# dohlee/diffab-pytorch

Hardware: AMD Instinct MI355X
Metric: CDR-residue denoise-steps/sec (K=128 patch) (higher is better)
Workload: dtype f32 (bf16x6 / fp16x3 split-precision products on the 16-bit matrix cores, fp32 accumulate; fp32-accurate, DESIGN section 4)

## Files before the change

### diffab-pytorch_amd/csrc/api.hip

```cpp
#include <atomic>
#include <cstring>
#include <mutex>
#include <vector>

#include "common.h"
#include "denoiser_internal.h"
#include "mlp_chain_tile.h"

namespace diffab {

static thread_local char g_err[512] = "";

void set_error(const char* fmt, ...) {
  va_list ap;
  va_start(ap, fmt);
  vsnprintf(g_err, sizeof(g_err), fmt, ap);
  va_end(ap);
}

namespace {
struct OrderState {
  std::recursive_mutex mu;
  hipStream_t last = nullptr;
  bool have = false;
// ... 132 lines not shown
  if (hipGetDevice(&dev) == hipSuccess) (void)hipDeviceGetAttribute(&ncu, hipDeviceAttributeMultiprocessorCount, dev);
  const int rounds = (d->B + ncu - 1) / ncu;
  return d->K == 128 && d->B >= ncu && static_cast<double>(d->B) >= 0.85 * rounds * ncu;
}

struct ForwardPlan {
  uint32_t flags;
  bool fold;
  bool b6;
  bool chain;
  bool persistent, fused_mlps;
  const float* pair_planes;
  const int* ctx_of_row;
  int n_ctx;
  const unsigned char* last_layer_tiles;
  float* res_emb;
};

static ForwardPlan plan_forward(const diffab_dims* d, uint32_t flags, const StepBuffers& b, const float* res_ctx, const float* pair_ctx,
                                float* res_emb, bool loop, const int* ctx_of_row = nullptr, int n_ctx = 0, unsigned char* tiles = nullptr) {
  const int rows = d->B * d->K, D = d->D;
  if (loop && !(flags & DIFFAB_FLAG_PAIR_F32)) flags |= DIFFAB_FLAG_PAIR_PLANES;
  ForwardPlan p{};
  p.flags = flags;
  p.fold = !(flags & DIFFAB_FLAG_FORCE_GENERIC) && fast_path_supported(d) && rowgemm128_ok(res_ctx, D, b.h1, D, rows, D);
  p.b6 = p.fold && use_b6_gemm(flags) && rowgemm128_b6_ok(res_ctx, D, b.h1, D, rows, D);
  p.chain = p.b6 && d->V <= 128;
  p.pair_planes = use_pair_planes(d, flags, pair_ctx, b) ? b.pair : nullptr;
  p.ctx_of_row = ctx_of_row;
  p.n_ctx = n_ctx;
  p.last_layer_tiles = tiles != nullptr && !(flags & DIFFAB_FLAG_ALL_ROWS) && p.fold && d->K % 16 == 0 && d->NL >= 2 ? tiles : nullptr;
  p.res_emb = res_emb;
  p.persistent = p.b6 && p.pair_planes != nullptr && ipa_module_persistent_supported(d) &&
                 ((flags & DIFFAB_FLAG_PERSISTENT_MODULE) || (loop && !(flags & DIFFAB_FLAG_MULTI_LAUNCH) && module_launch_fills_chip(d)));
  p.fused_mlps = p.persistent && p.chain && D == 128 && res_emb == nullptr;
  return p;
}

struct StepBias {
  const float* beta;
  const float* sched_beta;
  int t;
  const int* t_dev;
  float* beta_traj;
  int traj_rows;
};

static int prepare_forward(const diffab_dims* d, const diffab_denoiser_weights* w, const ForwardPlan& p, const StepBuffers& b,
                           const float* pair_ctx, const StepBias& bias, hipStream_t st) {
  if (p.fold)
// ... 62 lines not shown
  const int head_div = bias.beta_traj ? rows : d->K;
  if (p.chain) {
    for (int hd = 0; hd < 3; ++hd) {
      hpl[3 * hd] = mlp + (2 + 2 * hd) * mlp_planes_bytes();
      hpl[3 * hd + 1] = mlp + (3 + 2 * hd) * mlp_planes_bytes();
      hpl[3 * hd + 2] = mlp + (8 + hd) * mlp_planes_bytes();
      hbs[3 * hd] = bias.beta_traj ? bias.beta_traj + (static_cast<size_t>(hd) * bias.traj_rows + bias.t) * D
                                   : b.beta_tab + static_cast<size_t>(hd) * d->B * D;
      hbs[3 * hd + 1] = hw[hd]->b2;
      hbs[3 * hd + 2] = hw[hd]->b4;
    }
    if (int rc = make_mlp_chain_set(&head_set, 3, hpl, hbs, nullptr, head_div, 3, nout, outs, nout)) return rc;
  }
  if (p.persistent) {
    if (int rc = launch_ipa_module_persistent(d, b.hA, b.hB, O_t, x_t, b.ipa, b.planes, p.pair_planes, st, p.fused_mlps ? res_ctx : nullptr,
                                              &emb_set, &head_set, p.ctx_of_row, p.n_ctx, p.last_layer_tiles))
      return rc;
    cur = (d->NL & 1) ? b.hB : b.hA;
  }
  for (int l = 0; l < d->NL && !p.persistent; ++l) {
    const void* planes = p.b6 ? b.planes + l * ipa_layer_planes_bytes() : nullptr;
    if (int rc = ipa_layer_dispatch(d, &w->layers[l], cur, pair_ctx, O_t, x_t, nxt, b.ipa, p.flags, st, nullptr, nullptr, planes, p.pair_planes,
                                    false, l == d->NL - 1 ? p.last_layer_tiles : nullptr, p.ctx_of_row, p.n_ctx))
      return rc;
    float* tmp = cur; cur = nxt; nxt = tmp;
  }
  if (p.res_emb) DIFFAB_HIP_CHECK(hipMemcpyAsync(p.res_emb, cur, sizeof(float) * rows * D, hipMemcpyDeviceToDevice, st));
  if (p.chain) {
    if (!p.fused_mlps)
      if (int rc = launch_mlp_chains_b6(cur, D, 3, hpl, hbs, nullptr, head_div, 3, nout, outs, nout, rows, st)) return rc;
  } else if (p.fold) {
// ... 37 lines not shown
  float* outs[3] = {out_eps, tp.vbuf, tp.logits};
  const int nout[3] = {3, 3, d->V};
  for (int hd = 0; hd < 3; ++hd) {
    if (int rc = launch_linear(tp.cat3, D + 3, hw[hd]->w0, hw[hd]->b0, tp.t1[hd], D, rows, D, D + 3, true, st)) return rc;
    if (int rc = launch_linear(tp.t1[hd], D, hw[hd]->w2, hw[hd]->b2, tp.t2[hd], D, rows, D, D, true, st)) return rc;
    if (int rc = launch_linear(tp.t2[hd], D, hw[hd]->w4, hw[hd]->b4, outs[hd], nout[hd], rows, nout[hd], D, false, st)) return rc;
  }
  return launch_heads_finish(tp.vbuf, O_t, tp.logits, d->V, rows, out_O0, out_post, st);
}

constexpr int kTrajRows = 1025;
struct SampleBuffers {
  float *beta, *eps, *O0, *post;
  int* t_dev;
  unsigned char* tiles;
  float* beta_traj;
  int* ctx_of_row;
  float* res_ctx;
  void* step;
  size_t bytes;
};

static SampleBuffers carve_sample(const diffab_dims* d, void* ws, int n_pair = 0, bool mapped = false) {
  Carver c(ws);
  const size_t rows = static_cast<size_t>(d->B) * d->K;
  SampleBuffers s;
  s.beta = c.take<float>(d->B);
  s.eps = c.take<float>(rows * 3);
  s.O0 = c.take<float>(rows * 9);
  s.post = c.take<float>(rows * d->V);
  s.t_dev = c.take<int>(64);
  s.tiles = c.take<unsigned char>(static_cast<size_t>(d->B) * ((d->K + 15) / 16));
  s.beta_traj = c.take<float>(static_cast<size_t>(3) * kTrajRows * d->D);
  s.ctx_of_row = mapped ? c.take<int>(d->B) : nullptr;
  s.res_ctx = mapped ? c.take<float>(rows * d->D) : nullptr;
  const size_t step_bytes = carve_step(d, nullptr, n_pair).bytes;
  s.step = c.take<char>(step_bytes);
  s.bytes = c.bytes();
  return s;
}

struct ScoreBuffers {
  int* t_list;
  float* beta;
  int* ctx_of_row;
  int64_t* seq_t;
  float *x_t, *O_t, *eps, *eps_hat;
// ... 87 lines not shown

int diffab_debug_set_module_stagger(int32_t ticks_10ns, int32_t classes) {
  set_module_stagger(ticks_10ns, classes);
  return DIFFAB_OK;
}

int diffab_debug_set_module_stamps(void* device_buffer) {
  set_module_stamps(device_buffer);
  return DIFFAB_OK;
}

int diffab_debug_row_tiles(const uint8_t* gen_mask, int32_t B, int32_t K, uint8_t* tiles, void* stream) {
  StreamOrder order_(stream);
  DIFFAB_REQUIRE(gen_mask && tiles && B >= 1 && K >= 16 && K % 16 == 0, DIFFAB_ERR_ARG, "debug_row_tiles: need B >= 1 and K a multiple of 16");
  return launch_tiles_needed(gen_mask, B, K, tiles, as_stream(stream));
}

int diffab_debug_set_attn_variant(int32_t v) { return set_attn_variant(v); }

int diffab_debug_set_attn_stamps(void* device_buffer) {
  set_attn_stamps(device_buffer);
  return DIFFAB_OK;
}

int diffab_kernel_timer_enable(int on) {
  g_timer.on = on != 0;
  g_timer.used = 0;
  return DIFFAB_OK;
}

// ... 429 lines not shown
  const bool mapped = ctx_of_row != nullptr;
  int n_ctx = opt->n_ctx;
  bool identity = false;
  if (int rc = context_map_option(d, ctx_of_row, &n_ctx, &identity)) return rc;
  const SampleBuffers sb = carve_sample(d, workspace, n_ctx, mapped);
  DIFFAB_REQUIRE(workspace_bytes >= sb.bytes, DIFFAB_ERR_WORKSPACE, "sample_loop: workspace %zu < %zu bytes", workspace_bytes, sb.bytes);
  hipStream_t st = as_stream(stream);
  const int* ctx_dev = nullptr;
  if (!identity) {
    DIFFAB_HIP_CHECK(hipMemcpyAsync(sb.ctx_of_row, ctx_of_row, sizeof(int32_t) * d->B, hipMemcpyHostToDevice, st));
    if (int rc = launch_gather_rows(res_ctx, sb.ctx_of_row, d->B, static_cast<int64_t>(d->K) * d->D, sb.res_ctx, st)) return rc;
    ctx_dev = sb.ctx_of_row;
    res_ctx = sb.res_ctx;
  }
  const StepBuffers b0 = carve_step(d, sb.step, n_ctx);
  const ForwardPlan plan = plan_forward(d, flags, b0, res_ctx, pair_ctx, nullptr, true, ctx_dev, n_ctx, sb.tiles);
  StepBias bias{sb.beta, plan.fold ? s->beta : nullptr, 0, nullptr, nullptr, s->T + 1};
  if (plan.chain && s->T + 1 <= kTrajRows && !(flags & DIFFAB_FLAG_GRAPH_SAMPLER)) bias.beta_traj = sb.beta_traj;
  if (int rc = prepare_forward(d, w, plan, b0, pair_ctx, bias, st)) return rc;
  if (plan.last_layer_tiles)
    if (int rc = launch_tiles_needed(gen_mask, d->B, d->K, sb.tiles, st)) return rc;
  if (rec != nullptr) {
    DIFFAB_HIP_CHECK(hipMemcpyAsync(rec->slot_dev, rec->slot_of_step, sizeof(int32_t) * (s->T + 1), hipMemcpyHostToDevice, st));
    if (int rc = launch_record_fixed(uo.rec, seq, x, O, gen_mask, d->B, d->K, d->V, st)) return rc;
  }
  if (steps != nullptr)
    DIFFAB_HIP_CHECK(hipMemcpyAsync(steps->plan_dev, plan_host.data(), sizeof(int32_t) * plan_host.size(), hipMemcpyHostToDevice, st));
  if (steering != nullptr && steering->ancestors != nullptr)
    DIFFAB_HIP_CHECK(hipMemsetAsync(steering->ancestors, 0xFF, sizeof(int32_t) * static_cast<size_t>(s->T + 1) * d->B, st));
  auto one_step = [&](int t, const int* t_dev) -> int {
    if (!plan.fold)
      if (int rc = launch_fill_beta(s, t, d->B, sb.beta, st, t_dev)) return rc;
    StepBias step = bias;
    step.t = t;
    step.t_dev = t_dev;
    if (int rc = denoise_step(d, w, plan, step, seq, x, O, res_ctx, pair_ctx, sb.eps, nullptr, nullptr, nullptr, b0, st)) return rc;
// ... 126 lines not shown
```

### diffab-pytorch_amd/csrc/denoiser_fast.hip

```cpp
#include <cstdlib>
#include <type_traits>

#include "common.h"
#include "denoiser_internal.h"
#include "rowgemm_b6_tile.h"
#include "ipa_attn_tile.h"

namespace diffab {


constexpr int LBM = 128, LBK = 32, LLD = LBK + 4;

struct LinearSegs {
  const float* W[6];
  int n_end[6];
  int nseg;
};

template <int BN, bool RELU, bool VEC>
__global__ __launch_bounds__(256) void linear_mfma_kernel(const float* __restrict__ X, int ldx, LinearSegs segs,
                                                          const float* __restrict__ bias, float* __restrict__ Y, int ldy, int M, int N,
                                                          int Kd) {
  __shared__ __attribute__((aligned(16))) float As[LBM * LLD];
  __shared__ __attribute__((aligned(16))) float Bs[BN * LLD];
// ... 279 lines not shown
                                                            const unsigned char* __restrict__ tile_needed = nullptr,
                                                            const int* __restrict__ ctx_of_row = nullptr) {
  extern __shared__ __attribute__((aligned(16))) float S[];
  const int ntile = (MULTI ? NC_arg : 1) * NT;
  int b, tile;
  const unsigned bid = blockIdx.x;
  if ((B & 7) == 0) {
    const int xcd = bid & 7, slot = bid >> 3;
    b = (slot / ntile) * 8 + xcd;
    tile = slot % ntile;
  } else {
    b = bid / ntile;
    tile = bid % ntile;
  }
  if (tile_needed != nullptr && !tile_needed[b * ntile + tile]) return;
  ipa_attn_tile<NT, MULTI, PLANES, TAPE>(S, b, tile, bid, proj, e, R, t, Wb, gamma, feat, NC_arg, stamps, esc, tape_p, tape_d2, ctx_of_row);
}

static unsigned long long* g_attn_stamps = nullptr;
static bool g_pair_chain_off = false;
void set_pair_embed_fused(bool on);
int set_attn_variant(int v) {
  DIFFAB_REQUIRE((v & ~(4 | 64)) == 0, DIFFAB_ERR_ARG, "debug_set_attn_variant: %d has bits other than 4 and 64", v);
  set_pair_embed_fused(!(v & 4));
  g_pair_chain_off = (v & 64) != 0;
  return DIFFAB_OK;
}
bool pair_chain_bwd_enabled() { return !g_pair_chain_off; }
void set_attn_stamps(void* p) {
  g_attn_stamps = static_cast<unsigned long long*>(p);
}
// ... 242 lines not shown
```

### diffab-pytorch_amd/csrc/denoiser_internal.h

```cpp
#pragma once
#include "common.h"

namespace diffab {

int launch_linear_generic(const float* X, int ldx, const float* W, const float* bias, float* Y, int ldy, int M, int N, int Kd, bool relu,
                          hipStream_t st);
size_t ipa_generic_workspace_floats(const diffab_dims* d);
int ipa_layer_generic(const diffab_dims* d, const diffab_ipa_layer_weights* w, const float* x, const float* e, const float* R, const float* t,
                      float* y, float* ws, hipStream_t st, const int* ctx_of_row = nullptr);
int launch_embed_concat(const float* res_ctx, const float* emb, const int64_t* seq, int D, int64_t rows, float* out, hipStream_t st);
int launch_beta_concat(const float* h, const float* beta, int D, int K, int64_t rows, float* out, hipStream_t st);
int launch_heads_finish(const float* v, const float* O_t, const float* logits, int V, int64_t rows, float* O0, float* post, hipStream_t st);
int launch_proj_frames_f32(const float* x, const float* const* W6, const float* R, const float* t, float* proj, int rows, hipStream_t st);
int launch_losses_bwd(const float* post, const float* tpost, const float* eps, const float* teps, const float* O0, const float* tO,
                      const float* O_t, const float* v, const uint8_t* gm, const uint8_t* rm, const float* count, const float* up, int V,
                      int64_t rows, float* d_logits, float* d_eps, float* d_v, hipStream_t st);
int launch_heads_cotangent(const float* post, const float* c_post, const float* c_eps, const float* c_O0, const float* O_t, const float* v,
                           int V, int64_t rows, float* d_logits, float* d_eps, float* d_v, float* d_Ot, hipStream_t st);
int launch_ipa_frames_bwd(const float* proj, const float* dproj, int NP, int pt_col0, int n_pts, const float* feat, const float* dfeat, int F,
                          int ol_col0, int on_col0, int n_vpts, const float* R, const float* t, float* dR, float* dt, int rows,
                          hipStream_t st);

bool fast_path_supported(const diffab_dims* d);
size_t ipa_fast_workspace_floats(const diffab_dims* d);
// ... 50 lines not shown
size_t ipa_layer_h3_out_offset();
size_t ipa_layer_h3_wis_offset();
size_t rowgemm128_h3_planes_bytes(int Kd);
size_t proj_frames_h3_planes_bytes();
int launch_wsplit128_h3(const float* W, int ldw, int Kd, void* planes, float* wis, hipStream_t st, int nrows = 128);
int launch_pjsplit_h3(const float* const* W6, void* planes, float* wis, hipStream_t st);
int launch_rowgemm128_h3p(const float* X, int ldx, const void* planes, const float* wis, const float* bias, const int64_t* bias_idx, int bias_div,
                          float* Y, int ldy, int M, int Kd, bool relu, hipStream_t st, float* parts = nullptr);
int launch_proj_frames_h3p(const float* x, const void* planes, const float* wis, const float* R, const float* t, float* proj, int rows,
                           hipStream_t st);
int ipa_layer_split_weights(const diffab_ipa_layer_weights* w, void* planes, hipStream_t st);
bool ipa_module_persistent_supported(const diffab_dims* d);
int launch_ipa_module_persistent(const diffab_dims* d, float* xa, float* xb, const float* R, const float* t, float* ws, const void* planes,
                                 const float* pair_planes, hipStream_t st, const float* emb_X = nullptr, const MlpChainSet* emb = nullptr,
                                 const MlpChainSet* heads = nullptr, const int* ctx_of_row = nullptr, int n_ctx = 0,
                                 const unsigned char* last_layer_tiles = nullptr);
void set_module_stagger(int ticks, int classes);
void set_module_stamps(void* device_buffer);
int launch_fold_embed_table(const diffab_dims* d, const diffab_denoiser_weights* w, float* emb_tab, hipStream_t st);
int launch_fold_beta_table(const diffab_dims* d, const diffab_denoiser_weights* w, const float* beta, float* beta_tab, hipStream_t st,
                           const float* sched_beta = nullptr, int t = 0, const int* t_dev = nullptr);

bool pair_embed_fused_supported(const diffab_ctx_dims* d);
size_t pair_embed_fused_prep_floats(const diffab_ctx_dims* d);
int launch_pair_embed_fused(const diffab_ctx_dims* d, const diffab_pair_emb_weights* w, const int64_t* seq_idx, const float* distmat,
                            const float* xyz, const float* pairwise_dihedrals, const int64_t* residue_idx, int32_t residue_idx_batch_stride,
                            const int64_t* chain_idx, const float* atom_mask, const uint8_t* sequence_context_mask, float* out, float* prep,
                            float* tape_h1, float* tape_df, float* tape_m1, float* tape_m2, int64_t row0, int64_t nrows, hipStream_t st,
                            const float** coef_sp_out = nullptr);
int launch_softplus_table(const float* coefw, int n, float* out, hipStream_t st);

// ... 135 lines not shown
  SampleRecordDev rec;
  StepPlanDev plan;
  GuidanceDev guide;
  TemperatureDev temp;
  SteeringDev steer;
};
int launch_reverse_update_philox(const diffab_sched* s, const diffab_igso3* tab, int t, int64_t* seq, float* x, float* O,
                                 const float* eps_hat, float* O0_hat, float* post, const uint8_t* gm, uint64_t seed,
                                 int64_t first_patch, int B, int K, int V, hipStream_t st, const int* t_dev, const float* head_v,
                                 const float* head_logits, const UpdateOptions& o);
int check_guidance_terms(const diffab_sample_guidance* g, const char* who);
int launch_record_fixed(const SampleRecordDev& rec, const int64_t* seq, const float* x, const float* O, const uint8_t* gm, int B, int K, int V,
                        hipStream_t st);
int launch_fill_beta(const diffab_sched* s, int t, int B, float* out, hipStream_t st, const int* t_dev = nullptr);
int launch_tiles_needed(const uint8_t* gm, int B, int K, unsigned char* out, hipStream_t st);
int launch_gather_rows(const float* src, const int* ctx_of_row, int B, int64_t row_floats, float* out, hipStream_t st);
struct ScoreChunk {
  const int* t_list;
  int n_t, n_draws, K;
  int64_t q0;
  int rows, valid;
  uint32_t keep;
};
constexpr int kScoreCtxMax = 256;
struct ScoreCtxTable {
  int64_t r0;
  int ctx[kScoreCtxMax];
};
int launch_score_noise(const diffab_sched* s, const diffab_igso3* fwd, const ScoreChunk& c, const int64_t* seq0, const float* x0,
                       const float* O0, const uint8_t* gm, const int32_t* ctx_of_design, uint64_t seed, int64_t first_design, int64_t* s_t,
// ... 10 lines not shown
```

### diffab-pytorch_amd/csrc/diffusion_kernels.hip

```cpp
#include <cmath>

#include "common.h"
#include "denoiser_internal.h"
#include "guidance_row.h"
#include "philox.h"
#include "so3_math.h"

namespace diffab {

constexpr int kThreads = 256;
static inline int blocks_for(int64_t n) { return static_cast<int>((n + kThreads - 1) / kThreads); }
constexpr float kPiF = 3.14159265358979323846f;
constexpr double kPiD = 3.14159265358979323846;

__device__ inline int sched_index(int64_t t, int T) { return static_cast<int>(t < 0 ? t + (T + 1) : t); }

__global__ void so3_log_kernel(const float* __restrict__ R, float* __restrict__ S, int64_t n) {
  const int64_t i = blockIdx.x * static_cast<int64_t>(blockDim.x) + threadIdx.x;
  if (i >= n) return;
  float r[9], s[9];
#pragma unroll
  for (int k = 0; k < 9; ++k) r[k] = R[i * 9 + k];
  so3_log(r, s);
#pragma unroll
// ... 1225 lines not shown
  return DIFFAB_OK;
}
__global__ void tiles_needed_kernel(const uint8_t* __restrict__ gm, int64_t ntiles, unsigned char* __restrict__ out) {
  const int64_t i = blockIdx.x * static_cast<int64_t>(blockDim.x) + threadIdx.x;
  if (i >= ntiles) return;
  unsigned char any = 0;
  for (int r = 0; r < 16; ++r) any |= gm[i * 16 + r];
  out[i] = any != 0;
}
int launch_tiles_needed(const uint8_t* gm, int B, int K, unsigned char* out, hipStream_t st) {
  const int64_t n = static_cast<int64_t>(B) * (K / 16);
  hipLaunchKernelGGL(tiles_needed_kernel, dim3(static_cast<unsigned>((n + 255) / 256)), dim3(256), 0, st, gm, n, out);
  DIFFAB_LAUNCH_CHECK();
  return DIFFAB_OK;
}
__global__ void gather_rows_kernel(const float* __restrict__ src, const int* __restrict__ ctx_of_row, int64_t row_floats, int64_t n,
                                   float* __restrict__ out) {
  const int64_t i = blockIdx.x * static_cast<int64_t>(blockDim.x) + threadIdx.x;
  if (i >= n) return;
  const int64_t b = i / row_floats;
  out[i] = src[static_cast<int64_t>(ctx_of_row[b]) * row_floats + (i - b * row_floats)];
}
int launch_gather_rows(const float* src, const int* ctx_of_row, int B, int64_t row_floats, float* out, hipStream_t st) {
  const int64_t n = static_cast<int64_t>(B) * row_floats;
  hipLaunchKernelGGL(gather_rows_kernel, dim3(static_cast<unsigned>((n + 255) / 256)), dim3(256), 0, st, src, ctx_of_row, row_floats, n, out);
  DIFFAB_LAUNCH_CHECK();
  return DIFFAB_OK;
}
int launch_set_int(int* p, int v, hipStream_t st) {
  hipLaunchKernelGGL(set_int_kernel, dim3(1), dim3(1), 0, st, p, v);
// ... 425 lines not shown
```

### diffab-pytorch_amd/csrc/ipa_attn_tile.h

```cpp
#pragma once
#include <hip/hip_runtime.h>
#include <cmath>
#include <cstdint>

namespace diffab {

typedef float f32x4 __attribute__((ext_vector_type(4)));
typedef float f32x16 __attribute__((ext_vector_type(16)));
typedef float f32x2 __attribute__((ext_vector_type(2)));

#ifndef MEM_FENCE
#define MEM_FENCE() asm volatile("" ::: "memory")
#endif

constexpr int AH = 8, ADS = 32, AP = 8, AC = 64;
constexpr int ANP = 3 * AH * ADS + 3 * AH * AP * 3;
constexpr int AF = AH * ADS + AH * AC + AH * AP * 3 + AH * AP;
constexpr int OFF_QS = 0, OFF_KS = 256, OFF_VS = 512, OFF_GQ = 768, OFF_GK = 960, OFF_GV = 1152;
constexpr int FOFF_OS = 0, FOFF_OE = 256, FOFF_OL = 768, FOFF_ON = 960;
constexpr int TI = 16;


#define FAST_EXP(x) __expf(x)

// ... 35 lines not shown
  pre.gqr[0] = *reinterpret_cast<const f32x4*>(ug + lo.p0);
  pre.gqr[1] = *reinterpret_cast<const f32x4*>(ug + lo.p1);
}

template <bool PLANES, typename FP>
__device__ __forceinline__ void attn_shift_pair_rows(FP& e, FP& esc, const int* __restrict__ ctx_of_row, const int b, const int K) {
  if (ctx_of_row == nullptr) return;
  int c;
  asm volatile("s_load_dword %0, %1, 0x0\n\ts_waitcnt lgkmcnt(0)" : "=s"(c) : "s"(ctx_of_row + b) : "memory");
  const int64_t shift = static_cast<int64_t>(c - b) * K;
  e += shift * K * AC;
  if constexpr (PLANES) esc += 2 * shift;
}

template <int NT, bool MULTI, bool PLANES = false, bool TAPE = false>
__device__ __forceinline__ void ipa_attn_tile(float* __restrict__ S, const int b, const int tile, const unsigned stamp_id,
                                              const float* __restrict__ proj, const float* __restrict__ e,
                                              const float* __restrict__ R, const float* __restrict__ t,
                                              const float* __restrict__ Wb, const float* __restrict__ gamma,
                                              float* __restrict__ feat, int NC_arg,
                                              unsigned long long* __restrict__ stamps, const float* __restrict__ esc = nullptr,
                                              float* __restrict__ tape_p = nullptr, float* __restrict__ tape_d2 = nullptr,
                                              const int* __restrict__ ctx_of_row = nullptr) {
  static_assert(!PLANES || NT % 2 == 0, "the o_e product takes key tiles in pairs");
  static_assert(!TAPE || (!MULTI && !PLANES), "the tape form is the single-chunk fp32-pair kernel");
  const int NC = MULTI ? NC_arg : 1;
  constexpr int KC = NT * 16;
  const int K = NC * KC;
  auto stamp = [&](int k) {
    if (stamps != nullptr) {
      __builtin_amdgcn_sched_barrier(0);
#ifdef AT_STAMP_REALTIME
      const unsigned long long tnow = __builtin_amdgcn_s_memrealtime();
#else
      const unsigned long long tnow = __builtin_amdgcn_s_memtime();
#endif
      if ((threadIdx.x & 63) == 0) stamps[(static_cast<size_t>(stamp_id) * 8 + (threadIdx.x >> 6)) * 8 + k] = tnow;
      __builtin_amdgcn_sched_barrier(0);
    }
  };
  stamp(0);
  const int i0 = tile * TI;
  const int tid = threadIdx.x, lane0 = tid & 63, wv = __builtin_amdgcn_readfirstlane(tid >> 6);
  constexpr int HS = KC + 8, IS = AH * (KC + 8) + 8;
  const int64_t prow0 = static_cast<int64_t>(b) * K;
  attn_shift_pair_rows<PLANES>(e, esc, ctx_of_row, b, K);
  const float scale_t = 0.57735026918962576f;

  constexpr int KLD = 40, GLD = 28;
  constexpr int P1_TILE = 16 * KLD + 16 * GLD;
  constexpr int ELD = 72;
  constexpr int SCR_FLOATS = 2 * 16 * ELD;
  constexpr int E_LAG = MULTI ? 2 : 0;
  constexpr int E_EARLY = MULTI ? 1 : 2;
  float* scr = S + TI * IS + wv * SCR_FLOATS;
  float* st_fac = S + TI * IS + 8 * SCR_FLOATS;
  float* st_inv = st_fac + TI * AH;
// ... 574 lines not shown
```

### diffab-pytorch_amd/csrc/ipa_persistent.hip

```cpp
#include "common.h"
#include "denoiser_internal.h"
#define AT_STAMP_REALTIME 1
#include "ipa_attn_tile.h"
#include "proj_frames_h3_tile.h"
#include "rowgemm_h3_tile.h"
#include "mlp_chain_tile.h"

namespace diffab {

namespace {
constexpr size_t cmax(size_t a, size_t b) { return a > b ? a : b; }
constexpr size_t kModuleLdsBytes = cmax(cmax(ipa_attn_lds_bytes(8), static_cast<size_t>(kChainLdsBytes)),
                                        cmax(static_cast<size_t>(pjh3::PJ_LDS_BYTES), static_cast<size_t>(h3tile::lds_bytes<128>())));
constexpr size_t kXImageOffset = cmax(static_cast<size_t>(pjh3::PJ_LDS_BYTES), static_cast<size_t>(h3tile::lds_bytes<128>())) / 4;
static_assert(kXImageOffset * 4 + h3tile::y_lds_bytes<128>() <= kModuleLdsBytes, "module LDS: no room for the x image of the dense phases");
static_assert(kModuleLdsBytes <= 160 * 1024, "module LDS: one work-group per CU within gfx950's 160 KiB");
static_assert(kXImageOffset % 4 == 0, "x image: 16-byte aligned rows");

struct ModuleArgs {
  float* xa;
  float* xb;
  float* proj;
  float* feat;
  const float* pair;
  const float* esc;
  const int* ctx_of_row;
  const unsigned char* last_layer_tiles;
  const float* R;
  const float* t;
  const char* planes;
  size_t layer_stride, pj_off, out_off, wis_off, small_off;
  unsigned long long* stamps;
  const float* emb_X;
  MlpChainSet emb, heads;
  int B, NL;
  int stagger_ticks, stagger_classes;
};
}

__device__ __forceinline__ bool module_tile_needed(const unsigned char* __restrict__ map, const int idx) {
  unsigned w;
  asm volatile("s_load_dword %0, %1, 0x0\n\ts_waitcnt lgkmcnt(0)" : "=s"(w) : "s"(map + (idx & ~3)) : "memory");
  return ((w >> (8 * (idx & 3))) & 0xffu) != 0;
}

template <int KRES>
__global__ __launch_bounds__(512) void ipa_module_persistent_kernel(const ModuleArgs a) {
  extern __shared__ __attribute__((aligned(16))) float lds[];
  constexpr int K = KRES, NTILE = K / TI, DT = K / 128;
  static_assert(KRES == 128 || KRES == 256, "patch-resident module: K = 128 or 256");
  const int M = a.B * K;
  if (a.stagger_ticks > 0 && a.stagger_classes > 1) {
    const unsigned long long t0 = __builtin_amdgcn_s_memrealtime();
    const unsigned long long wait = static_cast<unsigned long long>((blockIdx.x >> 3) % a.stagger_classes) * a.stagger_ticks;
    while (__builtin_amdgcn_s_memrealtime() - t0 < wait) __builtin_amdgcn_s_sleep(32);
  }
  unsigned long long* pstamps = a.stamps ? a.stamps + static_cast<size_t>(a.B) * a.NL * NTILE * 64 : nullptr;
  auto pstamp = [&](int b, int l, int k) {
// ... 39 lines not shown
                                                             reinterpret_cast<const float*>(lp + a.wis_off), a.R, a.t, a.proj, M, 0, 0, 0,
                                                             lds + kXImageOffset);
        } else {
          pjh3::proj_frames_h3_tile<true, false>(reinterpret_cast<_Float16*>(lds), tid, b * DT + dt, 0, 1, xin,
                                                 reinterpret_cast<const _Float16*>(lp + a.pj_off), reinterpret_cast<const float*>(lp + a.wis_off),
                                                 a.R, a.t, a.proj, M);
        }
        if (dt + 1 < DT) {
          asm volatile("s_waitcnt vmcnt(0)" ::: "memory");
          __syncthreads();
        }
      }
      asm volatile("s_waitcnt vmcnt(0)" ::: "memory");
      __syncthreads();
      pstamp(b, l, 1);
      const unsigned char* needed = l + 1 == a.NL ? a.last_layer_tiles : nullptr;
#pragma unroll 1
      for (int tile = 0; tile < NTILE; ++tile) {
        if (needed != nullptr && !module_tile_needed(needed, b * NTILE + tile)) continue;
        ipa_attn_tile<8, (KRES > 128), true>(lds, b, tile, static_cast<unsigned>((b * a.NL + l) * NTILE + tile), a.proj, a.pair, a.R, a.t, small,
                                             small + 512, a.feat, K / 128, a.stamps, a.esc, nullptr, nullptr, a.ctx_of_row);
        asm volatile("s_waitcnt vmcnt(0)" ::: "memory");
        __syncthreads();
      }
      pstamp(b, l, 2);
#pragma unroll 1
      for (int dt = 0; dt < DT; ++dt) {
        int tid = threadIdx.x;
        asm volatile("" : "+v"(tid));
        if (KRES == 128)
          h3tile::rowgemm128_h3_tile<false, 128, false, true>(reinterpret_cast<_Float16*>(lds), tid, b, a.feat, AF,
                                                              reinterpret_cast<const _Float16*>(lp + a.out_off),
                                                              reinterpret_cast<const float*>(lp + a.wis_off) + ANP, small + 576, nullptr, 0,
                                                              l + 1 == a.NL ? xout : nullptr, 128, M, AF, 0, nullptr, lds + kXImageOffset);
        else
// ... 2 lines not shown
                                                 reinterpret_cast<const float*>(lp + a.wis_off) + ANP, small + 576, nullptr, 0, xout, 128, M, AF);
        if (dt + 1 < DT) {
          asm volatile("s_waitcnt vmcnt(0)" ::: "memory");
          __syncthreads();
        }
      }
      asm volatile("s_waitcnt vmcnt(0)" ::: "memory");
      __syncthreads();
      pstamp(b, l, 3);
    }
    if (a.emb_X != nullptr) {
      const float* xfin = (a.NL & 1) ? a.xb : a.xa;
#pragma unroll 1
      for (int hdt = 0; hdt < 3 * DT; ++hdt) {
        const int hd = hdt / DT, dt = hdt % DT;
        int tid = threadIdx.x;
        asm volatile("" : "+v"(tid));
#define HSEL(f) (hd == 0 ? a.heads.c[0].f : hd == 1 ? a.heads.c[1].f : a.heads.c[2].f)
        chaintile::mlp_chain_tile(reinterpret_cast<__bf16*>(lds), tid, b * DT + dt, xfin, 128, HSEL(planes[0]), HSEL(planes[1]), HSEL(planes[2]),
                                  HSEL(bias[0]), HSEL(bias[1]), HSEL(bias[2]), HSEL(bias_idx0), HSEL(bias_div0), 3, HSEL(n_out),
                                  hd == 0 ? a.heads.Y[0] : hd == 1 ? a.heads.Y[1] : a.heads.Y[2],
                                  hd == 0 ? a.heads.ldy[0] : hd == 1 ? a.heads.ldy[1] : a.heads.ldy[2], M);
#undef HSEL
        asm volatile("s_waitcnt vmcnt(0)" ::: "memory");
        __syncthreads();
      }
    }
  }
}

namespace {
int g_stagger_ticks = 1000, g_stagger_classes = 8;
unsigned long long* g_module_stamps = nullptr;
}
void set_module_stagger(int ticks, int classes) {
  g_stagger_ticks = ticks;
  g_stagger_classes = classes;
}
void set_module_stamps(void* p) { g_module_stamps = static_cast<unsigned long long*>(p); }

bool ipa_module_persistent_supported(const diffab_dims* d) {
  return fast_path_supported(d) && (d->K == 128 || d->K == 256) && d->NL >= 1;
}

int launch_ipa_module_persistent(const diffab_dims* d, float* xa, float* xb, const float* R, const float* t, float* ws, const void* planes,
                                 const float* pair_planes, hipStream_t st, const float* emb_X, const MlpChainSet* emb,
                                 const MlpChainSet* heads, const int* ctx_of_row, int n_ctx, const unsigned char* last_layer_tiles) {
  DIFFAB_REQUIRE(ipa_module_persistent_supported(d) && xa && xb && R && t && ws && planes && pair_planes, DIFFAB_ERR_ARG,
                 "ipa_module_persistent: unsupported operands");
  DIFFAB_REQUIRE((reinterpret_cast<uintptr_t>(last_layer_tiles) & 3) == 0, DIFFAB_ERR_ARG,
                 "ipa_module_persistent: the row-tile map must be 4-byte aligned");
  const size_t rows = static_cast<size_t>(d->B) * d->K;
  ModuleArgs a{};
  a.xa = xa;
  a.xb = xb;
  a.proj = ws;
  a.feat = ws + rows * ANP;
  a.pair = pair_planes + 64;
  a.esc = pair_row_scales(d, pair_planes, n_ctx);
  a.ctx_of_row = ctx_of_row;
  a.last_layer_tiles = last_layer_tiles;
  a.R = R;
  a.t = t;
  a.planes = static_cast<const char*>(planes);
  a.layer_stride = ipa_layer_planes_bytes();
  a.pj_off = ipa_layer_h3_pj_offset();
  a.out_off = ipa_layer_h3_out_offset();
  a.wis_off = ipa_layer_h3_wis_offset();
  a.small_off = ipa_layer_small_offset();
  a.stamps = g_module_stamps;
  if (emb_X != nullptr) {
    DIFFAB_REQUIRE(emb && heads && d->D == 128 && (reinterpret_cast<uintptr_t>(emb_X) & 15) == 0, DIFFAB_ERR_ARG,
                   "ipa_module_persistent: the fused MLP phases need both chain sets");
    a.emb_X = emb_X;
    a.emb = *emb;
    a.heads = *heads;
// ... 25 lines not shown
```

### diffab-pytorch_amd/csrc/mlp_chain_tile.h

```cpp
#pragma once
#include <hip/hip_runtime.h>
#include <cstdint>

#include "rowgemm_b6_tile.h"

namespace diffab {
struct MlpChain {
  const __bf16* planes[3];
  const float* bias[3];
  const int64_t* bias_idx0;
  int bias_div0;
  int nlayers;
  int n_out;
};
constexpr int kChainLdsBytes = 2 * 3 * 128 * b6tile::BK * 2 + 4 * 3 * 128 * b6tile::BK * 2;
struct MlpChainSet {
  MlpChain c[3];
  float* Y[3];
  int ldy[3];
};


namespace chaintile {
using b6tile::BK;
using b6tile::b6_off;
using b6tile::split3;
typedef float f32x4 __attribute__((ext_vector_type(4)));
typedef __bf16 bf16x8 __attribute__((ext_vector_type(8)));
typedef float f32x16 __attribute__((ext_vector_type(16)));
#define CHAIN_FENCE() asm volatile("" ::: "memory")

__device__ __forceinline__ void mlp_chain_tile(__bf16* cl, const int tid, const int tile_m, const float* __restrict__ X, int ldx,
                                               const __bf16* pl0, const __bf16* pl1, const __bf16* pl2, const float* bs0, const float* bs1,
                                               const float* bs2, const int64_t* bias_idx0, int bias_div0, int nlayers, int n_out,
                                               float* __restrict__ Y, int ldy, int M) {
  struct { const int64_t* bias_idx0; int bias_div0, nlayers, n_out; } ch{bias_idx0, bias_div0, nlayers, n_out};
  auto planes_of = [&](int L) { return L == 0 ? pl0 : L == 1 ? pl1 : pl2; };
  auto bias_of = [&](int L) { return L == 0 ? bs0 : L == 1 ? bs1 : bs2; };
  __bf16* Ws = cl;
  __bf16* img = cl + 2 * 3 * 128 * BK;
  const int lane = tid & 63, wv = tid >> 6;
  const int l31 = lane & 31, hk = lane >> 5, rw = wv & 3, cw = wv >> 2;
  const int m0 = tile_m * 128;
  typedef __bf16 bf16x4 __attribute__((ext_vector_type(4)));
  {
    const int xa_row = tid >> 3, xa_part = tid & 7;
    f32x4 xr[4][2];
#pragma unroll
    for (int j = 0; j < 2; ++j) {
      int row = m0 + xa_row + 64 * j;
      row = row < M ? row : M - 1;
      const float* src = X + static_cast<int64_t>(row) * ldx + 4 * xa_part;
#pragma unroll
      for (int c = 0; c < 4; ++c) xr[c][j] = *reinterpret_cast<const f32x4*>(src + c * BK);
    }
#pragma unroll
    for (int c = 0; c < 4; ++c)
#pragma unroll
      for (int j = 0; j < 2; ++j) {
        bf16x4 h, m, l;
#pragma unroll
        for (int e = 0; e < 4; ++e) {
          __bf16 hh, mm, ll;
          split3(xr[c][j][e], hh, mm, ll);
          h[e] = hh; m[e] = mm; l[e] = ll;
        }
        __bf16* dst = img + c * (3 * 128 * BK) + b6_off(xa_row + 64 * j, xa_part >> 1) + 4 * (xa_part & 1);
        *reinterpret_cast<bf16x4*>(dst) = h;
        *reinterpret_cast<bf16x4*>(dst + 128 * BK) = m;
        *reinterpret_cast<bf16x4*>(dst + 2 * 128 * BK) = l;
      }
  }
  int w_dst[3];
#pragma unroll
// ... 19 lines not shown
#pragma unroll
    for (int tt = 0; tt < 2; ++tt)
#pragma unroll
      for (int r = 0; r < 16; ++r) acc[tt][r] = 0.f;
    store_w(0);
    load_w(Wc, 1);
    CHAIN_FENCE();
    __syncthreads();
#pragma unroll 1
    for (int c = 0; c < 4; ++c) {
      const int buf = c & 1;
      const __bf16* al = img + c * (3 * 128 * BK) + a_off;
      const __bf16* wl = Ws + buf * (3 * 128 * BK) + w_off;
#pragma unroll
      for (int ks = 0; ks < 2; ++ks) {
        const int so = 8 * ((2 * ks + hk) ^ fx);
        bf16x8 a[3], b[2][3];
#pragma unroll
        for (int p = 0; p < 3; ++p) {
          a[p] = *reinterpret_cast<const bf16x8*>(al + (p * 128) * BK + so);
#pragma unroll
          for (int tt = 0; tt < 2; ++tt) b[tt][p] = *reinterpret_cast<const bf16x8*>(wl + (p * 128 + 32 * tt) * BK + so);
        }
#pragma unroll
        for (int term = 0; term < 6; ++term)
#pragma unroll
          for (int tt = 0; tt < 2; ++tt)
            acc[tt] = __builtin_amdgcn_mfma_f32_32x32x16_bf16(b[tt][TB[term]], a[TA[term]], acc[tt], 0, 0, 0);
      }
      if (c < 3) {
        store_w(buf ^ 1);
        if (c < 2) load_w(Wc, c + 2);
        else if (!last) load_w(planes_of(L + 1), 0);
        CHAIN_FENCE();
      }
      __syncthreads();
    }
    const bool table = L == 0 && (ch.bias_idx0 != nullptr || ch.bias_div0 > 0);
    const int lrow = 32 * rw + l31, row = m0 + lrow;
    const float* bl = bias_of(L);
    if (table) {
      const int rc = row < M ? row : M - 1;
      const int64_t bi = ch.bias_idx0 ? ch.bias_idx0[rc] : rc / ch.bias_div0;
      bl = bs0 + bi * 128;
    }
#pragma unroll
    for (int tt = 0; tt < 2; ++tt)
#pragma unroll
      for (int g4 = 0; g4 < 4; ++g4) {
        const int col = 64 * cw + 32 * tt + 8 * g4 + 4 * hk;
        f32x4 bv = {0.f, 0.f, 0.f, 0.f};
        if (bl && (table || !last || col + 3 < ch.n_out)) bv = *reinterpret_cast<const f32x4*>(bl + col);
// ... 34 lines not shown
```

### diffab-pytorch_amd/diffab_pytorch/_hip.py

```python
from __future__ import annotations

import ctypes as C
import os
from typing import Dict, Optional, Sequence

import torch

_HERE = os.path.dirname(os.path.abspath(__file__))
LIB_PATH = os.environ.get("DIFFAB_HIP_LIB") or os.path.join(os.path.dirname(_HERE), "lib", "libdiffab_hip.so")

FLAG_FORCE_GENERIC = 1
FLAG_PAIR_F32 = 64
FLAG_FP32_GEMM = 128
FLAG_PAIR_PLANES = 32
FLAG_GRAPH_SAMPLER = 16
FLAG_PERSISTENT_MODULE = 512
FLAG_MULTI_LAUNCH = 1024
FLAG_SKIP_UNUSED_ROWS = 256
FLAG_ALL_ROWS = 8192
FLAG_KEEP_STRUCTURE = 2048
FLAG_KEEP_SEQUENCE = 4096


class HipUnavailable(RuntimeError):
# ... 90 lines not shown
        super().__init__(struct_bytes=C.sizeof(type(self)), **{k: v for k, v in options.items() if v is not None})


_i32, _i64, _u32, _u64, _sz = C.c_int32, C.c_int64, C.c_uint32, C.c_uint64, C.c_size_t
_PD, _PS, _PI = C.POINTER(Dims), C.POINTER(Sched), C.POINTER(Igso3)
SYMBOLS = {
    "diffab_version": (C.c_char_p, []),
    "diffab_last_error": (C.c_char_p, []),
    "diffab_device_ok": (C.c_int, []),
    "diffab_kernel_timer_enable": (C.c_int, [C.c_int]),
    "diffab_debug_set_attn_stamps": (C.c_int, [_fp]),
    "diffab_debug_set_attn_variant": (C.c_int, [_i32]),
    "diffab_debug_set_module_stagger": (C.c_int, [_i32, _i32]),
    "diffab_debug_set_module_stamps": (C.c_int, [_fp]),
    "diffab_debug_row_tiles": (C.c_int, [_fp, _i32, _i32, _fp, _fp]),
    "diffab_set_stream_guard": (C.c_int, [C.c_int]),
    "diffab_debug_linear128": (C.c_int, [_fp, _fp, _fp, _fp, C.c_int64, C.c_int32, C.c_int32, _fp, C.c_size_t, _fp]),
    "diffab_debug_gemm_tn": (C.c_int, [_fp, _fp, _fp, _fp, C.c_int64, C.c_int32, C.c_int32, C.c_int32, _fp]),
    "diffab_debug_xstat128": (C.c_int, [_fp, _fp, _fp, C.c_int64, C.c_int32, C.c_int32, _fp, C.c_size_t, _fp]),
    "diffab_kernel_timer_read": (C.c_int, [C.POINTER(C.c_int64), C.POINTER(C.c_double)]),
    "diffab_so3_log": (C.c_int, [_fp, _fp, _i64, _fp]),
    "diffab_so3_exp": (C.c_int, [_fp, _fp, _i64, _fp]),
    "diffab_so3_matrix_to_rotvec": (C.c_int, [_fp, _fp, _i64, _fp]),
    "diffab_so3_rotvec_to_matrix": (C.c_int, [_fp, _fp, _i64, _fp]),
    "diffab_so3_scale_rot": (C.c_int, [_fp, _fp, _fp, _i64, _i64, _fp]),
    "diffab_igso3_table_build": (C.c_int, [_fp, _i32, _i32, _i32, _fp, _fp]),
    "diffab_igso3_table_build_accurate": (C.c_int, [_fp, _i32, _i32, _i32, _fp, _fp]),
    "diffab_igso3_cdf_build": (C.c_int, [_fp, _i32, _i32, _fp, _fp]),
    "diffab_igso3_sample": (C.c_int, [_PI, _fp, _i32, _i32, _fp, _fp, _fp, _fp, _fp, _fp]),
    "diffab_igso3_bins_without_replacement": (C.c_int, [_fp, _i32, _i32, _fp, _i32, _i32, _fp, _fp, _fp, C.c_float, _fp]),
# ... 194 lines not shown
```

### include/diffab_hip.h

```cpp
#ifndef DIFFAB_HIP_H
#define DIFFAB_HIP_H

#include <stddef.h>
#include <stdint.h>

#ifdef __cplusplus
extern "C" {
#endif

#define DIFFAB_OK 0
#define DIFFAB_ERR_ARG (-1)
#define DIFFAB_ERR_UNSUPPORTED (-2)
#define DIFFAB_ERR_HIP (-3)
#define DIFFAB_ERR_WORKSPACE (-4)

#define DIFFAB_FLAG_FORCE_GENERIC 1u

#define DIFFAB_FLAG_PAIR_PLANES 32u

#define DIFFAB_FLAG_PAIR_F32 64u
#define DIFFAB_FLAG_FP32_GEMM 128u

#define DIFFAB_FLAG_GRAPH_SAMPLER 16u
#define DIFFAB_FLAG_PERSISTENT_MODULE 512u
// ... 60 lines not shown
  const float* sigmas;
  const float* cdf;
  float sigma_threshold;
} diffab_igso3;

const char* diffab_version(void);
const char* diffab_last_error(void);
int diffab_device_ok(void);

int diffab_kernel_timer_enable(int on);
int diffab_debug_set_attn_stamps(void* device_buffer);
int diffab_debug_set_attn_variant(int32_t v);
int diffab_debug_set_module_stagger(int32_t ticks_10ns, int32_t classes);
int diffab_debug_set_module_stamps(void* device_buffer);
int diffab_debug_row_tiles(const uint8_t* gen_mask, int32_t B, int32_t K, uint8_t* tiles, void* stream);
int diffab_set_stream_guard(int on);
int diffab_debug_linear128(const float* X, const float* W, const float* bias, float* Y, int64_t M, int32_t Kd, int32_t mode, void* scratch,
                           size_t scratch_bytes, void* stream);
int diffab_debug_xstat128(const float* X, const float* W, float* Y, int64_t M, int32_t N, int32_t mode, void* scratch, size_t scratch_bytes,
                          void* stream);
int diffab_debug_gemm_tn(const float* A, const float* B, float* C, float* db, int64_t M, int32_t N1, int32_t N2, int32_t mode, void* stream);
int diffab_kernel_timer_read(int64_t* launches, double* total_ms);
int diffab_so3_log(const float* R, float* S, int64_t n, void* stream);
int diffab_so3_exp(const float* S, float* R, int64_t n, void* stream);
int diffab_so3_matrix_to_rotvec(const float* R, float* v, int64_t n, void* stream);
int diffab_so3_rotvec_to_matrix(const float* v, float* R, int64_t n, void* stream);
int diffab_so3_scale_rot(const float* R, const float* k, float* out, int64_t n, int64_t per_k, void* stream);

int diffab_igso3_table_build(const float* sigmas, int32_t n_sigmas, int32_t n_bins, int32_t num_iters, float* pdf, void* stream);
int diffab_igso3_table_build_accurate(const float* sigmas, int32_t n_sigmas, int32_t n_bins, int32_t num_iters, float* pdf,
// ... 333 lines not shown
```

Measured before the change: 14.72 million.

## Plan last-layer attention rows per batch and skip idle head-MLP slabs

Replaces the per-tile needed-flag map with a per-batch row plan. The plan lists 16-row windows that cover the generated (CDR) residues, plus a bitmask of 32-row slabs that contain generated rows. The persistent module's last IPA layer now runs attention only on those windows, which can start at any row, instead of on fixed 16-row tiles. The fused head MLP chain skips staging, MFMA and writeback for waves whose slab holds no generated rows. This trims wasted compute at the cost of an extra small kernel launch per sample, a changed wave-to-row mapping in the head tile, and some risk of mismatch between windows that overlap.

New measurement: 14.98 million (median of 6 runs). +1.8%, better.

```diff
diff --git a/diffab-pytorch_amd/csrc/api.hip b/diffab-pytorch_amd/csrc/api.hip
--- a/diffab-pytorch_amd/csrc/api.hip
+++ b/diffab-pytorch_amd/csrc/api.hip
@@ -170,11 +170,13 @@
   const int* ctx_of_row;
   int n_ctx;
   const unsigned char* last_layer_tiles;
+  const int* last_layer_rows;
   float* res_emb;
 };
 
 static ForwardPlan plan_forward(const diffab_dims* d, uint32_t flags, const StepBuffers& b, const float* res_ctx, const float* pair_ctx,
-                                float* res_emb, bool loop, const int* ctx_of_row = nullptr, int n_ctx = 0, unsigned char* tiles = nullptr) {
+                                float* res_emb, bool loop, const int* ctx_of_row = nullptr, int n_ctx = 0, unsigned char* tiles = nullptr,
+                                int* row_plan = nullptr) {
   const int rows = d->B * d->K, D = d->D;
   if (loop && !(flags & DIFFAB_FLAG_PAIR_F32)) flags |= DIFFAB_FLAG_PAIR_PLANES;
   ForwardPlan p{};
@@ -190,6 +192,7 @@
   p.persistent = p.b6 && p.pair_planes != nullptr && ipa_module_persistent_supported(d) &&
                  ((flags & DIFFAB_FLAG_PERSISTENT_MODULE) || (loop && !(flags & DIFFAB_FLAG_MULTI_LAUNCH) && module_launch_fills_chip(d)));
   p.fused_mlps = p.persistent && p.chain && D == 128 && res_emb == nullptr;
+  p.last_layer_rows = p.persistent && p.last_layer_tiles != nullptr ? row_plan : nullptr;
   return p;
 }
 
@@ -282,7 +285,7 @@
   }
   if (p.persistent) {
     if (int rc = launch_ipa_module_persistent(d, b.hA, b.hB, O_t, x_t, b.ipa, b.planes, p.pair_planes, st, p.fused_mlps ? res_ctx : nullptr,
-                                              &emb_set, &head_set, p.ctx_of_row, p.n_ctx, p.last_layer_tiles))
+                                              &emb_set, &head_set, p.ctx_of_row, p.n_ctx, p.last_layer_rows))
       return rc;
     cur = (d->NL & 1) ? b.hB : b.hA;
   }
@@ -350,6 +353,7 @@
   float *beta, *eps, *O0, *post;
   int* t_dev;
   unsigned char* tiles;
+  int* row_plan;
   float* beta_traj;
   int* ctx_of_row;
   float* res_ctx;
@@ -367,6 +371,7 @@
   s.post = c.take<float>(rows * d->V);
   s.t_dev = c.take<int>(64);
   s.tiles = c.take<unsigned char>(static_cast<size_t>(d->B) * ((d->K + 15) / 16));
+  s.row_plan = c.take<int>(static_cast<size_t>(d->B) * (2 + (d->K + 15) / 16));
   s.beta_traj = c.take<float>(static_cast<size_t>(3) * kTrajRows * d->D);
   s.ctx_of_row = mapped ? c.take<int>(d->B) : nullptr;
   s.res_ctx = mapped ? c.take<float>(rows * d->D) : nullptr;
@@ -484,6 +489,13 @@
   StreamOrder order_(stream);
   DIFFAB_REQUIRE(gen_mask && tiles && B >= 1 && K >= 16 && K % 16 == 0, DIFFAB_ERR_ARG, "debug_row_tiles: need B >= 1 and K a multiple of 16");
   return launch_tiles_needed(gen_mask, B, K, tiles, as_stream(stream));
+}
+
+int diffab_debug_row_plan(const uint8_t* gen_mask, int32_t B, int32_t K, int32_t* plan, void* stream) {
+  StreamOrder order_(stream);
+  DIFFAB_REQUIRE(gen_mask && plan && B >= 1 && K >= 16 && K <= 1024 && K % 16 == 0, DIFFAB_ERR_ARG,
+                 "debug_row_plan: need B >= 1 and K a multiple of 16 in 16 .. 1024");
+  return launch_row_plan(gen_mask, B, K, plan, as_stream(stream));
 }
 
 int diffab_debug_set_attn_variant(int32_t v) { return set_attn_variant(v); }
@@ -943,12 +955,14 @@
     res_ctx = sb.res_ctx;
   }
   const StepBuffers b0 = carve_step(d, sb.step, n_ctx);
-  const ForwardPlan plan = plan_forward(d, flags, b0, res_ctx, pair_ctx, nullptr, true, ctx_dev, n_ctx, sb.tiles);
+  const ForwardPlan plan = plan_forward(d, flags, b0, res_ctx, pair_ctx, nullptr, true, ctx_dev, n_ctx, sb.tiles, sb.row_plan);
   StepBias bias{sb.beta, plan.fold ? s->beta : nullptr, 0, nullptr, nullptr, s->T + 1};
   if (plan.chain && s->T + 1 <= kTrajRows && !(flags & DIFFAB_FLAG_GRAPH_SAMPLER)) bias.beta_traj = sb.beta_traj;
   if (int rc = prepare_forward(d, w, plan, b0, pair_ctx, bias, st)) return rc;
   if (plan.last_layer_tiles)
     if (int rc = launch_tiles_needed(gen_mask, d->B, d->K, sb.tiles, st)) return rc;
+  if (plan.last_layer_rows)
+    if (int rc = launch_row_plan(gen_mask, d->B, d->K, sb.row_plan, st)) return rc;
   if (rec != nullptr) {
     DIFFAB_HIP_CHECK(hipMemcpyAsync(rec->slot_dev, rec->slot_of_step, sizeof(int32_t) * (s->T + 1), hipMemcpyHostToDevice, st));
     if (int rc = launch_record_fixed(uo.rec, seq, x, O, gen_mask, d->B, d->K, d->V, st)) return rc;
diff --git a/diffab-pytorch_amd/csrc/denoiser_fast.hip b/diffab-pytorch_amd/csrc/denoiser_fast.hip
--- a/diffab-pytorch_amd/csrc/denoiser_fast.hip
+++ b/diffab-pytorch_amd/csrc/denoiser_fast.hip
@@ -317,7 +317,7 @@
     tile = bid % ntile;
   }
   if (tile_needed != nullptr && !tile_needed[b * ntile + tile]) return;
-  ipa_attn_tile<NT, MULTI, PLANES, TAPE>(S, b, tile, bid, proj, e, R, t, Wb, gamma, feat, NC_arg, stamps, esc, tape_p, tape_d2, ctx_of_row);
+  ipa_attn_tile<NT, MULTI, PLANES, TAPE>(S, b, tile * TI, bid, proj, e, R, t, Wb, gamma, feat, NC_arg, stamps, esc, tape_p, tape_d2, ctx_of_row);
 }
 
 static unsigned long long* g_attn_stamps = nullptr;
diff --git a/diffab-pytorch_amd/csrc/denoiser_internal.h b/diffab-pytorch_amd/csrc/denoiser_internal.h
--- a/diffab-pytorch_amd/csrc/denoiser_internal.h
+++ b/diffab-pytorch_amd/csrc/denoiser_internal.h
@@ -88,7 +88,7 @@
 int launch_ipa_module_persistent(const diffab_dims* d, float* xa, float* xb, const float* R, const float* t, float* ws, const void* planes,
                                  const float* pair_planes, hipStream_t st, const float* emb_X = nullptr, const MlpChainSet* emb = nullptr,
                                  const MlpChainSet* heads = nullptr, const int* ctx_of_row = nullptr, int n_ctx = 0,
-                                 const unsigned char* last_layer_tiles = nullptr);
+                                 const int* last_layer_rows = nullptr);
 void set_module_stagger(int ticks, int classes);
 void set_module_stamps(void* device_buffer);
 int launch_fold_embed_table(const diffab_dims* d, const diffab_denoiser_weights* w, float* emb_tab, hipStream_t st);
@@ -254,6 +254,8 @@
                         hipStream_t st);
 int launch_fill_beta(const diffab_sched* s, int t, int B, float* out, hipStream_t st, const int* t_dev = nullptr);
 int launch_tiles_needed(const uint8_t* gm, int B, int K, unsigned char* out, hipStream_t st);
+constexpr int row_plan_ints(int K) { return 2 + K / 16; }
+int launch_row_plan(const uint8_t* gm, int B, int K, int* out, hipStream_t st);
 int launch_gather_rows(const float* src, const int* ctx_of_row, int B, int64_t row_floats, float* out, hipStream_t st);
 struct ScoreChunk {
   const int* t_list;
diff --git a/diffab-pytorch_amd/csrc/diffusion_kernels.hip b/diffab-pytorch_amd/csrc/diffusion_kernels.hip
--- a/diffab-pytorch_amd/csrc/diffusion_kernels.hip
+++ b/diffab-pytorch_amd/csrc/diffusion_kernels.hip
@@ -1263,6 +1263,29 @@
   DIFFAB_LAUNCH_CHECK();
   return DIFFAB_OK;
 }
+__global__ void row_plan_kernel(const uint8_t* __restrict__ gm, int B, int K, int* __restrict__ out) {
+  const int b = blockIdx.x * blockDim.x + threadIdx.x;
+  if (b >= B) return;
+  int* p = out + static_cast<int64_t>(b) * row_plan_ints(K);
+  int n = 0, covered = 0;
+  unsigned slabs = 0;
+  for (int i = 0; i < K; ++i) {
+    if (!gm[static_cast<int64_t>(b) * K + i]) continue;
+    slabs |= 1u << (i >> 5);
+    if (i < covered) continue;
+    const int s = i < K - 16 ? i : K - 16;
+    p[2 + n++] = s;
+    covered = s + 16;
+  }
+  for (int j = n; j < K / 16; ++j) p[2 + j] = -1;
+  p[0] = n;
+  p[1] = static_cast<int>(slabs);
+}
+int launch_row_plan(const uint8_t* gm, int B, int K, int* out, hipStream_t st) {
+  hipLaunchKernelGGL(row_plan_kernel, dim3(static_cast<unsigned>((B + 63) / 64)), dim3(64), 0, st, gm, B, K, out);
+  DIFFAB_LAUNCH_CHECK();
+  return DIFFAB_OK;
+}
 __global__ void gather_rows_kernel(const float* __restrict__ src, const int* __restrict__ ctx_of_row, int64_t row_floats, int64_t n,
                                    float* __restrict__ out) {
   const int64_t i = blockIdx.x * static_cast<int64_t>(blockDim.x) + threadIdx.x;
diff --git a/diffab-pytorch_amd/csrc/ipa_attn_tile.h b/diffab-pytorch_amd/csrc/ipa_attn_tile.h
--- a/diffab-pytorch_amd/csrc/ipa_attn_tile.h
+++ b/diffab-pytorch_amd/csrc/ipa_attn_tile.h
@@ -73,7 +73,7 @@
 }
 
 template <int NT, bool MULTI, bool PLANES = false, bool TAPE = false>
-__device__ __forceinline__ void ipa_attn_tile(float* __restrict__ S, const int b, const int tile, const unsigned stamp_id,
+__device__ __forceinline__ void ipa_attn_tile(float* __restrict__ S, const int b, const int i0, const unsigned stamp_id,
                                               const float* __restrict__ proj, const float* __restrict__ e,
                                               const float* __restrict__ R, const float* __restrict__ t,
                                               const float* __restrict__ Wb, const float* __restrict__ gamma,
@@ -99,7 +99,6 @@
     }
   };
   stamp(0);
-  const int i0 = tile * TI;
   const int tid = threadIdx.x, lane0 = tid & 63, wv = __builtin_amdgcn_readfirstlane(tid >> 6);
   constexpr int HS = KC + 8, IS = AH * (KC + 8) + 8;
   const int64_t prow0 = static_cast<int64_t>(b) * K;
diff --git a/diffab-pytorch_amd/csrc/ipa_persistent.hip b/diffab-pytorch_amd/csrc/ipa_persistent.hip
--- a/diffab-pytorch_amd/csrc/ipa_persistent.hip
+++ b/diffab-pytorch_amd/csrc/ipa_persistent.hip
@@ -25,7 +25,7 @@
   const float* pair;
   const float* esc;
   const int* ctx_of_row;
-  const unsigned char* last_layer_tiles;
+  const int* last_layer_rows;
   const float* R;
   const float* t;
   const char* planes;
@@ -38,10 +38,10 @@
 };
 }
 
-__device__ __forceinline__ bool module_tile_needed(const unsigned char* __restrict__ map, const int idx) {
-  unsigned w;
-  asm volatile("s_load_dword %0, %1, 0x0\n\ts_waitcnt lgkmcnt(0)" : "=s"(w) : "s"(map + (idx & ~3)) : "memory");
-  return ((w >> (8 * (idx & 3))) & 0xffu) != 0;
+__device__ __forceinline__ int module_plan_word(const int* __restrict__ plan, const int idx) {
+  int w;
+  asm volatile("s_load_dword %0, %1, 0x0\n\ts_waitcnt lgkmcnt(0)" : "=s"(w) : "s"(plan + idx) : "memory");
+  return w;
 }
 
 template <int KRES>
@@ -111,11 +111,12 @@
       asm volatile("s_waitcnt vmcnt(0)" ::: "memory");
       __syncthreads();
       pstamp(b, l, 1);
-      const unsigned char* needed = l + 1 == a.NL ? a.last_layer_tiles : nullptr;
-#pragma unroll 1
-      for (int tile = 0; tile < NTILE; ++tile) {
-        if (needed != nullptr && !module_tile_needed(needed, b * NTILE + tile)) continue;
-        ipa_attn_tile<8, (KRES > 128), true>(lds, b, tile, static_cast<unsigned>((b * a.NL + l) * NTILE + tile), a.proj, a.pair, a.R, a.t, small,
+      const int* rows = l + 1 == a.NL ? a.last_layer_rows : nullptr;
+      const int n_items = rows != nullptr ? module_plan_word(rows, b * (2 + NTILE)) : NTILE;
+#pragma unroll 1
+      for (int item = 0; item < n_items; ++item) {
+        const int i0 = rows != nullptr ? module_plan_word(rows, b * (2 + NTILE) + 2 + item) : item * TI;
+        ipa_attn_tile<8, (KRES > 128), true>(lds, b, i0, static_cast<unsigned>((b * a.NL + l) * NTILE + item), a.proj, a.pair, a.R, a.t, small,
                                              small + 512, a.feat, K / 128, a.stamps, a.esc, nullptr, nullptr, a.ctx_of_row);
         asm volatile("s_waitcnt vmcnt(0)" ::: "memory");
         __syncthreads();
@@ -148,17 +149,22 @@
 #pragma unroll 1
       for (int hdt = 0; hdt < 3 * DT; ++hdt) {
         const int hd = hdt / DT, dt = hdt % DT;
+        const unsigned hslabs =
+            a.last_layer_rows != nullptr ? static_cast<unsigned>(module_plan_word(a.last_layer_rows, b * (2 + NTILE) + 1)) : ~0u;
+        const unsigned tslabs = (hslabs >> (4 * dt)) & 15u;
+        if (tslabs == 0) continue;
         int tid = threadIdx.x;
         asm volatile("" : "+v"(tid));
 #define HSEL(f) (hd == 0 ? a.heads.c[0].f : hd == 1 ? a.heads.c[1].f : a.heads.c[2].f)
-        chaintile::mlp_chain_tile(reinterpret_cast<__bf16*>(lds), tid, b * DT + dt, xfin, 128, HSEL(planes[0]), HSEL(planes[1]), HSEL(planes[2]),
+        chaintile::mlp_chain_tile<true>(reinterpret_cast<__bf16*>(lds), tid, b * DT + dt, xfin, 128, HSEL(planes[0]), HSEL(planes[1]), HSEL(planes[2]),
                                   HSEL(bias[0]), HSEL(bias[1]), HSEL(bias[2]), HSEL(bias_idx0), HSEL(bias_div0), 3, HSEL(n_out),
                                   hd == 0 ? a.heads.Y[0] : hd == 1 ? a.heads.Y[1] : a.heads.Y[2],
-                                  hd == 0 ? a.heads.ldy[0] : hd == 1 ? a.heads.ldy[1] : a.heads.ldy[2], M);
+                                  hd == 0 ? a.heads.ldy[0] : hd == 1 ? a.heads.ldy[1] : a.heads.ldy[2], M, tslabs);
 #undef HSEL
         asm volatile("s_waitcnt vmcnt(0)" ::: "memory");
         __syncthreads();
       }
+      if (pstamps != nullptr && threadIdx.x == 0) pstamps[static_cast<size_t>(a.B) * a.NL * 4 + b] = __builtin_amdgcn_s_memrealtime();
     }
   }
 }
@@ -179,11 +185,11 @@
 
 int launch_ipa_module_persistent(const diffab_dims* d, float* xa, float* xb, const float* R, const float* t, float* ws, const void* planes,
                                  const float* pair_planes, hipStream_t st, const float* emb_X, const MlpChainSet* emb,
-                                 const MlpChainSet* heads, const int* ctx_of_row, int n_ctx, const unsigned char* last_layer_tiles) {
+                                 const MlpChainSet* heads, const int* ctx_of_row, int n_ctx, const int* last_layer_rows) {
   DIFFAB_REQUIRE(ipa_module_persistent_supported(d) && xa && xb && R && t && ws && planes && pair_planes, DIFFAB_ERR_ARG,
                  "ipa_module_persistent: unsupported operands");
-  DIFFAB_REQUIRE((reinterpret_cast<uintptr_t>(last_layer_tiles) & 3) == 0, DIFFAB_ERR_ARG,
-                 "ipa_module_persistent: the row-tile map must be 4-byte aligned");
+  DIFFAB_REQUIRE((reinterpret_cast<uintptr_t>(last_layer_rows) & 3) == 0, DIFFAB_ERR_ARG,
+                 "ipa_module_persistent: the row plan must be 4-byte aligned");
   const size_t rows = static_cast<size_t>(d->B) * d->K;
   ModuleArgs a{};
   a.xa = xa;
@@ -193,7 +199,7 @@
   a.pair = pair_planes + 64;
   a.esc = pair_row_scales(d, pair_planes, n_ctx);
   a.ctx_of_row = ctx_of_row;
-  a.last_layer_tiles = last_layer_tiles;
+  a.last_layer_rows = last_layer_rows;
   a.R = R;
   a.t = t;
   a.planes = static_cast<const char*>(planes);
diff --git a/diffab-pytorch_amd/csrc/mlp_chain_tile.h b/diffab-pytorch_amd/csrc/mlp_chain_tile.h
--- a/diffab-pytorch_amd/csrc/mlp_chain_tile.h
+++ b/diffab-pytorch_amd/csrc/mlp_chain_tile.h
@@ -30,24 +30,30 @@
 typedef float f32x16 __attribute__((ext_vector_type(16)));
 #define CHAIN_FENCE() asm volatile("" ::: "memory")
 
+template <bool SPREAD = false>
 __device__ __forceinline__ void mlp_chain_tile(__bf16* cl, const int tid, const int tile_m, const float* __restrict__ X, int ldx,
                                                const __bf16* pl0, const __bf16* pl1, const __bf16* pl2, const float* bs0, const float* bs1,
                                                const float* bs2, const int64_t* bias_idx0, int bias_div0, int nlayers, int n_out,
-                                               float* __restrict__ Y, int ldy, int M) {
+                                               float* __restrict__ Y, int ldy, int M, const unsigned slabs = ~0u) {
   struct { const int64_t* bias_idx0; int bias_div0, nlayers, n_out; } ch{bias_idx0, bias_div0, nlayers, n_out};
   auto planes_of = [&](int L) { return L == 0 ? pl0 : L == 1 ? pl1 : pl2; };
   auto bias_of = [&](int L) { return L == 0 ? bs0 : L == 1 ? bs1 : bs2; };
   __bf16* Ws = cl;
   __bf16* img = cl + 2 * 3 * 128 * BK;
   const int lane = tid & 63, wv = tid >> 6;
-  const int l31 = lane & 31, hk = lane >> 5, rw = wv & 3, cw = wv >> 2;
+  const int l31 = lane & 31, hk = lane >> 5;
+  const int rw = SPREAD ? wv >> 1 : wv & 3, cw = SPREAD ? wv & 1 : wv >> 2;
   const int m0 = tile_m * 128;
+  const int wv_u = __builtin_amdgcn_readfirstlane(wv);
+  const bool wanted = (slabs >> (SPREAD ? wv_u >> 1 : wv_u & 3)) & 1u;
   typedef __bf16 bf16x4 __attribute__((ext_vector_type(4)));
   {
     const int xa_row = tid >> 3, xa_part = tid & 7;
     f32x4 xr[4][2];
+    const bool stage[2] = {((slabs >> (wv_u >> 2)) & 1u) != 0, ((slabs >> (2 + (wv_u >> 2))) & 1u) != 0};
 #pragma unroll
     for (int j = 0; j < 2; ++j) {
+      if (!stage[j]) continue;
       int row = m0 + xa_row + 64 * j;
       row = row < M ? row : M - 1;
       const float* src = X + static_cast<int64_t>(row) * ldx + 4 * xa_part;
@@ -58,6 +64,7 @@
     for (int c = 0; c < 4; ++c)
 #pragma unroll
       for (int j = 0; j < 2; ++j) {
+        if (!stage[j]) continue;
         bf16x4 h, m, l;
 #pragma unroll
         for (int e = 0; e < 4; ++e) {
@@ -107,6 +114,7 @@
       const __bf16* wl = Ws + buf * (3 * 128 * BK) + w_off;
 #pragma unroll
       for (int ks = 0; ks < 2; ++ks) {
+        if (!wanted) break;
         const int so = 8 * ((2 * ks + hk) ^ fx);
         bf16x8 a[3], b[2][3];
 #pragma unroll
@@ -129,6 +137,7 @@
       }
       __syncthreads();
     }
+    if (!wanted) continue;
     const bool table = L == 0 && (ch.bias_idx0 != nullptr || ch.bias_div0 > 0);
     const int lrow = 32 * rw + l31, row = m0 + lrow;
     const float* bl = bias_of(L);
diff --git a/diffab-pytorch_amd/diffab_pytorch/_hip.py b/diffab-pytorch_amd/diffab_pytorch/_hip.py
--- a/diffab-pytorch_amd/diffab_pytorch/_hip.py
+++ b/diffab-pytorch_amd/diffab_pytorch/_hip.py
@@ -128,6 +128,7 @@
     "diffab_debug_set_module_stagger": (C.c_int, [_i32, _i32]),
     "diffab_debug_set_module_stamps": (C.c_int, [_fp]),
     "diffab_debug_row_tiles": (C.c_int, [_fp, _i32, _i32, _fp, _fp]),
+    "diffab_debug_row_plan": (C.c_int, [_fp, _i32, _i32, _fp, _fp]),
     "diffab_set_stream_guard": (C.c_int, [C.c_int]),
     "diffab_debug_linear128": (C.c_int, [_fp, _fp, _fp, _fp, C.c_int64, C.c_int32, C.c_int32, _fp, C.c_size_t, _fp]),
     "diffab_debug_gemm_tn": (C.c_int, [_fp, _fp, _fp, _fp, C.c_int64, C.c_int32, C.c_int32, C.c_int32, _fp]),
diff --git a/include/diffab_hip.h b/include/diffab_hip.h
--- a/include/diffab_hip.h
+++ b/include/diffab_hip.h
@@ -98,6 +98,7 @@
 int diffab_debug_set_module_stagger(int32_t ticks_10ns, int32_t classes);
 int diffab_debug_set_module_stamps(void* device_buffer);
 int diffab_debug_row_tiles(const uint8_t* gen_mask, int32_t B, int32_t K, uint8_t* tiles, void* stream);
+int diffab_debug_row_plan(const uint8_t* gen_mask, int32_t B, int32_t K, int32_t* plan, void* stream);
 int diffab_set_stream_guard(int on);
 int diffab_debug_linear128(const float* X, const float* W, const float* bias, float* Y, int64_t M, int32_t Kd, int32_t mode, void* scratch,
                            size_t scratch_bytes, void* stream);
```
